# microsoft/hyperspace

Measured on NVIDIA H100. Metric: createIndex rows/sec, higher is better.
Workload: dtype int64

## Files before the change

hyperspace_b200/csrc/device_utils.cuh:

```cuda
#pragma once
#include <cuda_runtime.h>

#include <cstdint>

#ifndef HS_HD
#ifdef __CUDACC__
#define HS_HD __host__ __device__ __forceinline__
#else
#define HS_HD inline
#endif
#endif

namespace hs {

HS_HD uint32_t rotl32(uint32_t x, int r) { return (x << r) | (x >> (32 - r)); }
HS_HD uint32_t mm3_mix_k1(uint32_t k1) {
  k1 *= 0xcc9e2d51u;
  k1 = rotl32(k1, 15);
  k1 *= 0x1b873593u;
  return k1;
}
HS_HD uint32_t mm3_mix_h1(uint32_t h1, uint32_t k1) {
  h1 ^= k1;
  h1 = rotl32(h1, 13);
// ... 199 lines not shown
        "{\n\t"
        ".reg .pred p;\n\t"
        ".reg .b32 t;\n\t"
        "and.b32 t, %2, %3;\n\t"
        "setp.ne.u32 p, t, 0;\n\t"
        "vote.sync.ballot.b32 %0, p, 0xffffffff;\n\t"
        "selp.b32 %1, 0, 0xffffffff, p;\n\t"
        "}"
        : "=r"(m), "=r"(x)
        : "r"(v), "r"(1u << b));
    peers &= m ^ x;
  }
  return peers;
}

__device__ __forceinline__ uint32_t block_exclusive_scan(uint32_t x, uint32_t* warp_sums, uint32_t* total) {
  const unsigned lane = threadIdx.x & 31, warp = threadIdx.x >> 5, nwarps = (blockDim.x + 31) >> 5;
  uint32_t incl = x;
#pragma unroll
  for (int o = 1; o < 32; o <<= 1) {
    uint32_t y = __shfl_up_sync(0xffffffffu, incl, o);
    if (lane >= (unsigned)o) incl += y;
  }
  __syncthreads();
  if (lane == 31) warp_sums[warp] = incl;
  __syncthreads();
  if (warp == 0) {
    uint32_t w = lane < nwarps ? warp_sums[lane] : 0;
    uint32_t wi = w;
#pragma unroll
// ... 17 lines not shown
```

hyperspace_b200/csrc/engine.cu:

```cuda
#include <fcntl.h>
#include <sys/stat.h>
#include <unistd.h>

#include <algorithm>
#include <array>
#include <cmath>
#include <map>
#include <random>

#include "device_utils.cuh"
#include "engine.h"

namespace hs {

std::string make_uuid() {
  std::random_device rd;
  std::mt19937_64 gen(((uint64_t)rd() << 32) ^ rd());
  uint64_t a = gen(), b = gen();
  char buf[40];
  snprintf(buf, sizeof buf, "%08x-%04x-4%03x-%04x-%012llx", (unsigned)(a >> 32), (unsigned)((a >> 16) & 0xffff),
           (unsigned)(a & 0xfff), (unsigned)(0x8000 | ((b >> 48) & 0x3fff)), (unsigned long long)(b & 0xffffffffffffull));
  return buf;
}

// ... 905 lines not shown
    int nbytes = 0, fourth_from_top = 0;
    for (int b = 7, seen = 0; b >= 0; b--)
      if ((varying >> (8 * b)) & 0xff) {
        nbytes++;
        if (++seen == want_bytes) fourth_from_top = b;
      }
    static const bool full_sort_only = getenv("HS_FULL_SORT") != nullptr;
    const RawKeyColumn raw{kc.data.get(), kc.type, kc.width};
    const RawKeyColumn* first_src = from_raw ? &raw : nullptr;
    if (from_raw && (varying == 0 || nrows == 0)) {
      launch_iota_u32(ctx, perm, nrows);
      launch_encode_keys(ctx, kc.data.get(), kc.type, nullptr, nrows, keys, d_or_and.get());
      first_src = nullptr;
    }
    const bool lsd_only = getenv("HS_LSD_SORT") != nullptr;
    if (first_src && !kc.has_nulls && !lsd_only && !full_sort_only) {
      bool local_done = false;
      if (max_bucket <= (uint64_t)kLocalSortCap) {
        segmented_sort_local(ctx, out->bucket_offsets.data(), num_buckets, raw, out->keys.get(), out->perm.get());
        local_done = true;
      } else if (nbytes > 2 && max_bucket <= (uint64_t)(0.85 * 256 * kLocalSortCap)) {
        const int shift = std::max(0, 63 - __builtin_clzll(varying) - 7);
        local_done = segmented_sort_msd_local(ctx, &out->plan, raw, shift, out->keys.get(), out->keys_alt.get(),
                                              out->perm.get(), out->perm_alt.get());
      }
      if (local_done) {
        keys = out->keys.get();
        perm = out->perm.get();
        keys_alt = out->keys_alt.get();
        perm_alt = out->perm_alt.get();
        sort_deferred = defer_settle && nkeys == 1;
        continue;
      }
    }
    if (nbytes > want_bytes && !full_sort_only) {
      const uint64_t high_mask = ~0ull << (8 * fourth_from_top);
      const uint64_t low_mask = ~high_mask;
      segmented_sort_pairs(ctx, &out->plan, keys, keys_alt, perm, perm_alt, varying & high_mask, first_src);
      out->d_fix_flag.alloc(ctx, 1);
// ... 727 lines not shown
```

hyperspace_b200/csrc/kernels.h:

```cpp
#pragma once
#include "hs_common.h"

namespace hs {

struct ChunkDesc {
  const uint8_t* data;
  uint64_t size;
  int64_t num_values;
  int64_t row_base;
  int32_t col;
  int32_t phys_type;
  int32_t max_def;
  int32_t file_index;
  int32_t codec;
  int32_t pad;
};

struct PageDesc {
  const uint8_t* data;
  const uint8_t* dict;
  int64_t first_row;
  int32_t dict_count;
  int32_t size;
  int32_t num_values;
// ... 145 lines not shown
  Buf<uint64_t> seg_start;
  Buf<uint32_t> tile_hist;
  Buf<uint32_t> tile_dst;
  std::vector<uint32_t> h_seg_tile_begin;
};
void build_sort_plan(hs_ctx* ctx, const uint64_t* seg_offsets, int nseg, SortPlan* plan);
struct RawKeyColumn {
  const void* data;
  int type, width;
};
void segmented_sort_pairs(hs_ctx* ctx, SortPlan* plan, uint64_t*& keys, uint64_t*& keys_alt, uint32_t*& vals,
                          uint32_t*& vals_alt, uint64_t bit_mask, const RawKeyColumn* first_pass_source = nullptr);
void launch_fix_runs(hs_ctx* ctx, SortPlan* plan, uint64_t* keys, uint32_t* vals, uint64_t high_mask, uint64_t low_mask,
                     uint32_t max_run, uint32_t* d_flag);
constexpr int kLocalSortCap = 12288;
struct LocalSortItem {
  uint32_t start, count;
};
void segmented_sort_local(hs_ctx* ctx, const uint64_t* seg_offsets, int nseg, const RawKeyColumn& raw, uint64_t* keys,
                          uint32_t* vals);
bool segmented_sort_msd_local(hs_ctx* ctx, SortPlan* plan, const RawKeyColumn& raw, int shift, uint64_t* keys,
                              uint64_t* keys_alt, uint32_t* vals, uint32_t* vals_alt);
void segmented_sort_pass_by_table(hs_ctx* ctx, SortPlan* plan, uint64_t*& keys, uint64_t*& keys_alt, uint32_t*& vals,
                                  uint32_t*& vals_alt, const uint8_t* digits);

struct GatherColumn {
  const void* src;
  const uint64_t* sorted_keys;
  int32_t key_type;
  int32_t width;
  const uint64_t* page_value_offset;
};
void launch_gather_encode(hs_ctx* ctx, const SortTile* tiles, int64_t ntiles, const uint64_t* seg_start,
                          const uint32_t* perm, const GatherColumn& col, const uint32_t* bucket_page_begin,
                          int64_t rows_per_page, uint8_t* arena);
void launch_tile_valid_counts(hs_ctx* ctx, const SortTile* tiles, int64_t ntiles, const uint32_t* perm,
                              const uint8_t* valid, uint32_t* counts);
// ... 79 lines not shown
```

hyperspace_b200/csrc/radix_sort.cu:

```cuda
#include "device_utils.cuh"
#include "kernels.h"

namespace hs {

namespace {

constexpr int kThreads = 512;
constexpr int kWarps = kThreads / 32;
constexpr int kItems = kSortTile / kThreads;
constexpr int kWarpRows = kSortTile / kWarps;
constexpr int kChunkTiles = 128;
constexpr int kHistThreads = 256;

struct SortChunk {
  uint32_t seg;
  uint32_t tile_begin, tile_end;
};

struct DigitShift {
  int shift;
  __device__ __forceinline__ uint32_t operator()(uint64_t key, uint32_t) const { return (uint32_t)(key >> shift) & 255u; }
};
struct DigitTable {
  const uint8_t* table;
  __device__ __forceinline__ uint32_t operator()(uint64_t, uint32_t val) const { return table[val]; }
};

struct SrcPairs {
  const uint64_t* __restrict__ keys;
  const uint32_t* __restrict__ vals;
  __device__ __forceinline__ void load(uint64_t p, uint64_t& k, uint32_t& v) const {
    k = keys[p];
    v = vals[p];
  }
};
template <int TYPE>
struct SrcRaw {
  const void* __restrict__ raw;
  __device__ __forceinline__ void load(uint64_t p, uint64_t& k, uint32_t& v) const {
    const uint64_t r = (TYPE == HS_TYPE_INT64 || TYPE == HS_TYPE_DOUBLE) ? ((const uint64_t*)raw)[p]
                                                                          : (uint64_t)((const uint32_t*)raw)[p];
    k = sort_encode(TYPE, r);
    v = (uint32_t)p;
  }
};

template <typename Src, typename Digit>
__global__ void __launch_bounds__(kHistThreads) k_sort_hist(const SortTile* __restrict__ tiles, Src src, Digit digit,
                                                         uint32_t* __restrict__ tile_hist) {
  __shared__ uint32_t s_hist[256];
  s_hist[threadIdx.x] = 0;
  __syncthreads();
  const SortTile t = tiles[blockIdx.x];
  for (uint32_t i = threadIdx.x; i < t.count; i += kHistThreads) {
    uint64_t k;
    uint32_t v;
    src.load(t.start + i, k, v);
    atomicAdd(&s_hist[digit(k, v)], 1u);
  }
  __syncthreads();
  tile_hist[(size_t)blockIdx.x * 256 + threadIdx.x] = s_hist[threadIdx.x];
}

__global__ void __launch_bounds__(256) k_seg_chunk_sums(const SortChunk* __restrict__ chunks,
                                                         const uint32_t* __restrict__ tile_hist,
                                                         uint32_t* __restrict__ chunk_sums) {
  const SortChunk c = chunks[blockIdx.x];
  uint32_t s = 0;
  for (uint32_t t = c.tile_begin; t < c.tile_end; t++) s += tile_hist[(size_t)t * 256 + threadIdx.x];
  chunk_sums[(size_t)blockIdx.x * 256 + threadIdx.x] = s;
}

__global__ void __launch_bounds__(256) k_seg_scan(const uint32_t* __restrict__ seg_chunk_begin,
                                                   const uint64_t* __restrict__ seg_start,
                                                   uint32_t* __restrict__ chunk_sums, uint32_t* __restrict__ digit_base) {
  __shared__ uint32_t warp_sums[40];
  const uint32_t seg = blockIdx.x;
  const uint32_t c0 = seg_chunk_begin[seg], c1 = seg_chunk_begin[seg + 1];
  uint32_t tot = 0;
  for (uint32_t c = c0; c < c1; c++) {
    const uint32_t v = chunk_sums[(size_t)c * 256 + threadIdx.x];
    chunk_sums[(size_t)c * 256 + threadIdx.x] = tot;
    tot += v;
  }
  const uint32_t dbase = block_exclusive_scan(tot, warp_sums, nullptr) + (uint32_t)seg_start[seg];
  if (digit_base) digit_base[(size_t)seg * 256 + threadIdx.x] = dbase;
  for (uint32_t c = c0; c < c1; c++) chunk_sums[(size_t)c * 256 + threadIdx.x] += dbase;
}

__global__ void __launch_bounds__(1024) k_seg_apply(const SortChunk* __restrict__ chunks,
                                                     const uint32_t* __restrict__ tile_hist,
                                                     uint32_t* __restrict__ tile_dst,
                                                     const uint32_t* __restrict__ chunk_sums) {
  __shared__ uint32_t s_group[4][256];
  const SortChunk c = chunks[blockIdx.x];
  const uint32_t d = threadIdx.x & 255, g = threadIdx.x >> 8;
  const uint32_t n = c.tile_end - c.tile_begin;
  const uint32_t per = (n + 3) / 4;
  const uint32_t t0 = c.tile_begin + min(g * per, n), t1 = c.tile_begin + min((g + 1) * per, n);
  uint32_t s = 0;
#pragma unroll 8
  for (uint32_t t = t0; t < t1; t++) s += tile_hist[(size_t)t * 256 + d];
  s_group[g][d] = s;
  __syncthreads();
  uint32_t run = chunk_sums[(size_t)blockIdx.x * 256 + d];
  for (uint32_t gg = 0; gg < g; gg++) run += s_group[gg][d];
#pragma unroll 8
  for (uint32_t t = t0; t < t1; t++) {
    const uint32_t v = tile_hist[(size_t)t * 256 + d];
    tile_dst[(size_t)t * 256 + d] = run;
    run += v;
  }
}

struct ScatterShared {
  uint64_t keys[kSortTile];
  uint32_t vals[kSortTile];
  uint16_t cnt[kWarps][256];
  uint32_t out_adj[256];
  uint32_t warp_sums[40];
};

template <typename Src, typename Digit>
__global__ void __launch_bounds__(kThreads, 2) k_sort_scatter(const SortTile* __restrict__ tiles, Src src, Digit digit,
                                                               const uint32_t* __restrict__ tile_dst,
                                                               uint64_t* __restrict__ out_keys,
                                                               uint32_t* __restrict__ out_vals) {
  extern __shared__ __align__(16) uint8_t smem_raw[];
  ScatterShared& sm = *reinterpret_cast<ScatterShared*>(smem_raw);
  const uint32_t warp = threadIdx.x >> 5, lane = threadIdx.x & 31;
  const unsigned lt = (1u << lane) - 1;
  {
    uint32_t* z = reinterpret_cast<uint32_t*>(&sm.cnt[0][0]);
#pragma unroll
    for (int i = 0; i < kWarps * 256 / 2 / kThreads; i++) z[threadIdx.x + i * kThreads] = 0;
  }
  const SortTile t = tiles[blockIdx.x];
  uint32_t dst0 = 0;
  if (threadIdx.x < 256) dst0 = tile_dst[(size_t)blockIdx.x * 256 + threadIdx.x];
  const uint32_t first = warp * kWarpRows + lane;
  const uint64_t p0 = t.start + first;
  uint64_t k[kItems];
  uint32_t v[kItems];
  uint32_t bin[kItems];
#pragma unroll
  for (int j = 0; j < kItems; j++) {
    const bool a = first + j * 32 < t.count;
    k[j] = ~0ull;
    v[j] = 0;
    if (a) src.load(p0 + j * 32, k[j], v[j]);
    bin[j] = a ? digit(k[j], v[j]) : 255u;
  }
  __syncthreads();
  uint16_t* cnt = sm.cnt[warp];
  uint32_t rank[kItems];
#pragma unroll
  for (int j = 0; j < kItems; j++) {
    const unsigned peers = match_any_full<8>(bin[j]);
    const uint32_t before = __popc(peers & lt);
    const uint32_t pre = cnt[bin[j]];
    __syncwarp();
    if (before == 0) cnt[bin[j]] = (uint16_t)(pre + __popc(peers));
    __syncwarp();
    rank[j] = pre + before;
  }
  __syncthreads();
  uint32_t total = 0;
  if (threadIdx.x < 256) {
#pragma unroll
    for (int w = 0; w < kWarps; w++) total += sm.cnt[w][threadIdx.x];
  }
  const uint32_t start = block_exclusive_scan(total, sm.warp_sums, nullptr);
  if (threadIdx.x < 256) {
    uint32_t run = start;
#pragma unroll
    for (int w = 0; w < kWarps; w++) {
      const uint16_t c = sm.cnt[w][threadIdx.x];
      sm.cnt[w][threadIdx.x] = (uint16_t)run;
      run += c;
    }
    sm.out_adj[threadIdx.x] = dst0 - start;
  }
  __syncthreads();
#pragma unroll
  for (int j = 0; j < kItems; j++) {
    const uint32_t pos = cnt[bin[j]] + rank[j];
    sm.keys[pos] = k[j];
    sm.vals[pos] = v[j];
// ... 110 lines not shown
      if (b == a) continue;
      const uint32_t va = vals[p + a];
      for (uint32_t c = a; c > b; c--) {
        const uint64_t kc = sk[c - 1];
        sk[c] = kc;
        keys[p + c] = kc;
        vals[p + c] = vals[p + c - 1];
      }
      sk[b] = ka;
      keys[p + b] = ka;
      vals[p + b] = va;
    }
  }
}

constexpr int kLocalThreads = 1024;
constexpr int kLocalWarps = kLocalThreads / 32;
constexpr int kLocalItems = kLocalSortCap / kLocalThreads;
constexpr int kLocalWarpRows = kLocalSortCap / kLocalWarps;
constexpr uint32_t kLocalMaxRun = 64;
static_assert(kLocalSortCap % kLocalThreads == 0 && kLocalSortCap <= 65536, "slot numbers are 16-bit");

struct LocalShared {
  uint64_t keys[kLocalSortCap];
  uint32_t vals[kLocalSortCap];
  uint16_t slot[kLocalSortCap];
  uint16_t cnt[kLocalWarps][256];
  uint32_t warp_sums[40];
  unsigned long long or_bits, and_bits;
  uint32_t long_run;
};

__device__ __forceinline__ void local_pass(LocalShared& sm, uint32_t count, int shift) {
  const uint32_t warp = threadIdx.x >> 5, lane = threadIdx.x & 31;
  const unsigned lt = (1u << lane) - 1;
  {
    uint32_t* z = reinterpret_cast<uint32_t*>(&sm.cnt[0][0]);
#pragma unroll
    for (int i = 0; i < kLocalWarps * 256 / 2 / kLocalThreads; i++) z[threadIdx.x + i * kLocalThreads] = 0;
  }
  const uint32_t first = warp * kLocalWarpRows + lane;
  uint32_t slot_bin[kLocalItems], rank[kLocalItems];
#pragma unroll
  for (int j = 0; j < kLocalItems; j++) {
    const uint32_t pos = first + j * 32;
    const uint32_t s = pos < count ? sm.slot[pos] : pos;
    slot_bin[j] = s << 8 | (pos < count ? (uint32_t)(sm.keys[s] >> shift) & 255u : 255u);
  }
  __syncthreads();
  uint16_t* cnt = sm.cnt[warp];
#pragma unroll
  for (int j = 0; j < kLocalItems; j++) {
    rank[j] = 0;
    if (warp * kLocalWarpRows + j * 32 < count) {
      const uint32_t bin = slot_bin[j] & 255u;
      const unsigned peers = match_any_full<8>(bin);
      const uint32_t before = __popc(peers & lt);
      const uint32_t pre = cnt[bin];
      __syncwarp();
      if (before == 0) cnt[bin] = (uint16_t)(pre + __popc(peers));
      __syncwarp();
      rank[j] = pre + before;
    }
  }
  __syncthreads();
  uint32_t total = 0;
  if (threadIdx.x < 256) {
#pragma unroll
    for (int w = 0; w < kLocalWarps; w++) total += sm.cnt[w][threadIdx.x];
  }
  const uint32_t start = block_exclusive_scan(total, sm.warp_sums, nullptr);
  if (threadIdx.x < 256) {
    uint32_t run = start;
#pragma unroll
    for (int w = 0; w < kLocalWarps; w++) {
      const uint16_t c = sm.cnt[w][threadIdx.x];
      sm.cnt[w][threadIdx.x] = (uint16_t)run;
      run += c;
    }
  }
  __syncthreads();
#pragma unroll
  for (int j = 0; j < kLocalItems; j++)
    if (warp * kLocalWarpRows + j * 32 < count) sm.slot[cnt[slot_bin[j] & 255u] + rank[j]] = (uint16_t)(slot_bin[j] >> 8);
  __syncthreads();
}

template <typename Src>
__global__ void __launch_bounds__(kLocalThreads, 1) k_local_sort(const LocalSortItem* __restrict__ items, Src src,
                                                                 uint64_t* __restrict__ out_keys,
                                                                 uint32_t* __restrict__ out_vals) {
  extern __shared__ __align__(16) uint8_t smem_raw[];
  LocalShared& sm = *reinterpret_cast<LocalShared*>(smem_raw);
  const LocalSortItem it = items[blockIdx.x];
  const uint32_t count = it.count;
  if (threadIdx.x == 0) {
    sm.or_bits = 0;
    sm.and_bits = ~0ull;
    sm.long_run = 0;
  }
  uint64_t k_or = 0, k_and = ~0ull;
  constexpr int kHalf = kLocalItems / 2;
#pragma unroll 1
  for (int h = 0; h < 2; h++) {
    uint64_t k[kHalf];
    uint32_t v[kHalf];
#pragma unroll
    for (int j = 0; j < kHalf; j++) {
      const uint32_t i = (h * kHalf + j) * kLocalThreads + threadIdx.x;
      if (i < count) src.load((uint64_t)it.start + i, k[j], v[j]);
    }
#pragma unroll
    for (int j = 0; j < kHalf; j++) {
      const uint32_t i = (h * kHalf + j) * kLocalThreads + threadIdx.x;
      if (i < count) {
        sm.keys[i] = k[j];
        sm.vals[i] = v[j];
        sm.slot[i] = (uint16_t)i;
        k_or |= k[j];
        k_and &= k[j];
      }
    }
  }
#pragma unroll
  for (int o = 16; o > 0; o >>= 1) {
    k_or |= __shfl_xor_sync(0xffffffffu, k_or, o);
    k_and &= __shfl_xor_sync(0xffffffffu, k_and, o);
  }
  __syncthreads();
  if ((threadIdx.x & 31) == 0) {
    atomicOr(&sm.or_bits, k_or);
    atomicAnd(&sm.and_bits, k_and);
  }
  __syncthreads();
  const uint64_t varying = sm.or_bits ^ sm.and_bits;
  if (varying != 0) {
    const int top = 63 - __clzll((long long)varying);
    int pbits = 1;
    while ((1u << pbits) < 2 * count) pbits++;
    const int ndig = (min(pbits, top + 1) + 7) / 8;
    const int low = max(0, top + 1 - 8 * ndig);
    for (int d = ndig - 1; d >= 0; d--) {
      const int shift = max(0, top + 1 - 8 * (d + 1));
      if ((varying >> shift) & 0xff) local_pass(sm, count, shift);
    }
    const uint64_t high_mask = ~0ull << low;
    if (varying & ~high_mask) {
      for (uint32_t i = threadIdx.x; i < count; i += kLocalThreads) {
        const uint64_t kh = sm.keys[sm.slot[i]] & high_mask;
        if (i > 0 && (sm.keys[sm.slot[i - 1]] & high_mask) == kh) continue;
        if (i + 1 >= count || (sm.keys[sm.slot[i + 1]] & high_mask) != kh) continue;
        uint32_t len = 2;
        while (i + len < count && len <= kLocalMaxRun && (sm.keys[sm.slot[i + len]] & high_mask) == kh) len++;
        if (len > kLocalMaxRun) {
          sm.long_run = 1;
          continue;
        }
        uint16_t* s = sm.slot + i;
        for (uint32_t a = 1; a < len; a++) {
          const uint16_t sa = s[a];
          const uint64_t ka = sm.keys[sa];
          uint32_t b = a;
          while (b > 0 && sm.keys[s[b - 1]] > ka) {
            s[b] = s[b - 1];
            b--;
          }
          s[b] = sa;
        }
      }
      __syncthreads();
      if (sm.long_run) {
        for (uint32_t i = threadIdx.x; i < count; i += kLocalThreads) sm.slot[i] = (uint16_t)i;
        __syncthreads();
        for (int shift = 0; shift < 64; shift += 8)
          if ((varying >> shift) & 0xff) local_pass(sm, count, shift);
      }
    }
  }
  __syncthreads();
#pragma unroll
  for (int j = 0; j < kLocalItems; j++) {
    const uint32_t i = j * kLocalThreads + threadIdx.x;
    if (i < count) {
      const uint32_t s = sm.slot[i];
      out_keys[(uint64_t)it.start + i] = sm.keys[s];
      out_vals[(uint64_t)it.start + i] = sm.vals[s];
    }
  }
}

template <typename Src>
void launch_local_sort(hs_ctx* ctx, const std::vector<LocalSortItem>& items, Src src, uint64_t* out_keys,
                       uint32_t* out_vals) {
  if (items.empty()) return;
  Buf<LocalSortItem> d_items(ctx, items.size());
  copy_h2d(ctx, d_items.get(), items.data(), items.size() * sizeof(LocalSortItem));
  static DeviceOnce attr_once;
  bool& attr = attr_once(ctx->device);
  if (!attr) {
    HS_CUDA(cudaFuncSetAttribute(k_local_sort<Src>, cudaFuncAttributeMaxDynamicSharedMemorySize, (int)sizeof(LocalShared)));
    attr = true;
  }
  KernelScope _ks(ctx, "k_local_sort");
  k_local_sort<Src><<<(unsigned)items.size(), kLocalThreads, sizeof(LocalShared), ctx->stream>>>(d_items.get(), src,
                                                                                                 out_keys, out_vals);
  HS_LAUNCH_CHECK(ctx);
}

template <typename Src, typename Digit>
void run_hist(hs_ctx* ctx, SortPlan* plan, const SortChunk* chunks, int64_t nchunks, const uint32_t* seg_chunk_begin,
              uint32_t* chunk_sums, Src src, Digit digit, uint32_t* digit_base) {
  {
    KernelScope _ks(ctx, "k_sort_hist");
    k_sort_hist<Src, Digit><<<(unsigned)plan->ntiles, kHistThreads, 0, ctx->stream>>>(plan->tiles.get(), src, digit,
                                                                                 plan->tile_hist.get());
    HS_LAUNCH_CHECK(ctx);
  }
  KernelScope _ks(ctx, "k_seg_scan");
  k_seg_chunk_sums<<<(unsigned)nchunks, 256, 0, ctx->stream>>>(chunks, plan->tile_hist.get(), chunk_sums);
  HS_LAUNCH_CHECK(ctx);
  k_seg_scan<<<(unsigned)plan->nseg, 256, 0, ctx->stream>>>(seg_chunk_begin, plan->seg_start.get(), chunk_sums, digit_base);
  HS_LAUNCH_CHECK(ctx);
}

template <typename Src, typename Digit>
void run_scatter(hs_ctx* ctx, SortPlan* plan, const SortChunk* chunks, int64_t nchunks, uint32_t* chunk_sums, Src src,
                 uint64_t* out_keys, uint32_t* out_vals, Digit digit) {
  {
    KernelScope _ks(ctx, "k_seg_scan");
    k_seg_apply<<<(unsigned)nchunks, 1024, 0, ctx->stream>>>(chunks, plan->tile_hist.get(), plan->tile_dst.get(), chunk_sums);
    HS_LAUNCH_CHECK(ctx);
  }
  static DeviceOnce attr_once;
  bool& attr = attr_once(ctx->device);
  if (!attr) {
    HS_CUDA(cudaFuncSetAttribute(k_sort_scatter<Src, Digit>, cudaFuncAttributeMaxDynamicSharedMemorySize,
                                 (int)sizeof(ScatterShared)));
    attr = true;
  }
  KernelScope _ks(ctx, "k_sort_scatter");
  k_sort_scatter<Src, Digit><<<(unsigned)plan->ntiles, kThreads, sizeof(ScatterShared), ctx->stream>>>(
      plan->tiles.get(), src, digit, plan->tile_dst.get(), out_keys, out_vals);
  HS_LAUNCH_CHECK(ctx);
}

template <typename Src, typename Digit>
void run_pass(hs_ctx* ctx, SortPlan* plan, const SortChunk* chunks, int64_t nchunks, const uint32_t* seg_chunk_begin,
              uint32_t* chunk_sums, Src src, uint64_t* out_keys, uint32_t* out_vals, Digit digit) {
  run_hist(ctx, plan, chunks, nchunks, seg_chunk_begin, chunk_sums, src, digit, nullptr);
  run_scatter(ctx, plan, chunks, nchunks, chunk_sums, src, out_keys, out_vals, digit);
}

struct ChunkPlan {
  Buf<SortChunk> chunks;
  Buf<uint32_t> seg_chunk_begin;
  Buf<uint32_t> chunk_sums;
  int64_t nchunks = 0;
};

ChunkPlan build_chunks(hs_ctx* ctx, const std::vector<uint32_t>& seg_tile_begin) {
  ChunkPlan cp;
  const int nseg = (int)seg_tile_begin.size() - 1;
  std::vector<SortChunk> chunks;
  std::vector<uint32_t> scb(nseg + 1);
  for (int s = 0; s < nseg; s++) {
    scb[s] = (uint32_t)chunks.size();
    for (uint32_t t = seg_tile_begin[s]; t < seg_tile_begin[s + 1]; t += kChunkTiles)
      chunks.push_back(SortChunk{(uint32_t)s, t, std::min<uint32_t>(t + kChunkTiles, seg_tile_begin[s + 1])});
  }
  scb[nseg] = (uint32_t)chunks.size();
  cp.nchunks = (int64_t)chunks.size();
  cp.chunks.alloc(ctx, std::max<size_t>(1, chunks.size()));
  cp.seg_chunk_begin.alloc(ctx, scb.size());
  cp.chunk_sums.alloc(ctx, std::max<size_t>(1, chunks.size()) * 256);
  if (!chunks.empty())
    copy_h2d(ctx, cp.chunks.get(), chunks.data(), chunks.size() * sizeof(SortChunk));
  copy_h2d(ctx, cp.seg_chunk_begin.get(), scb.data(), scb.size() * 4);
  return cp;
}

}

__global__ void k_build_tiles(const uint64_t* __restrict__ seg_start, const uint32_t* __restrict__ seg_tile_begin,
                              SortTile* __restrict__ tiles) {
  const uint32_t s = blockIdx.x;
  const uint64_t b = seg_start[s], e = seg_start[s + 1];
  const uint32_t t0 = seg_tile_begin[s], nt = seg_tile_begin[s + 1] - t0;
  for (uint32_t i = threadIdx.x; i < nt; i += blockDim.x) {
    const uint64_t p = b + (uint64_t)i * kSortTile;
// ... 71 lines not shown
    case HS_TYPE_FLOAT: f(SrcRaw<HS_TYPE_FLOAT>{raw.data}); break;
    case HS_TYPE_DOUBLE: f(SrcRaw<HS_TYPE_DOUBLE>{raw.data}); break;
    default: fail(HS_EUNSUPPORTED, "sort: key type %d", raw.type);
  }
}
}

void segmented_sort_local(hs_ctx* ctx, const uint64_t* seg_offsets, int nseg, const RawKeyColumn& raw, uint64_t* keys,
                          uint32_t* vals) {
  std::vector<LocalSortItem> items;
  for (int s = 0; s < nseg; s++) {
    const uint64_t n = seg_offsets[s + 1] - seg_offsets[s];
    if (n > (uint64_t)kLocalSortCap) fail(HS_EINVAL, "segmented_sort_local: segment of %llu rows", (unsigned long long)n);
    if (n) items.push_back(LocalSortItem{(uint32_t)seg_offsets[s], (uint32_t)n});
  }
  with_raw_source(raw, [&](auto src) { launch_local_sort(ctx, items, src, keys, vals); });
}

bool segmented_sort_msd_local(hs_ctx* ctx, SortPlan* plan, const RawKeyColumn& raw, int shift, uint64_t* keys,
                              uint64_t* keys_alt, uint32_t* vals, uint32_t* vals_alt) {
  if (plan->ntiles == 0) return false;
  ChunkPlan cp = build_chunks(ctx, plan->h_seg_tile_begin);
  const size_t nsub = (size_t)plan->nseg * 256;
  Buf<uint32_t> d_base(ctx, nsub);
  const DigitShift digit{shift};
  with_raw_source(raw, [&](auto src) {
    run_hist(ctx, plan, cp.chunks.get(), cp.nchunks, cp.seg_chunk_begin.get(), cp.chunk_sums.get(), src, digit, d_base.get());
  });
  std::vector<uint32_t> base(nsub + 1);
  copy_d2h(ctx, base.data(), d_base.get(), nsub * 4);
  sync_stream(ctx);
  base[nsub] = (uint32_t)plan->n;
  std::vector<LocalSortItem> items;
  for (int s = 0; s < plan->nseg; s++) {
    LocalSortItem cur{base[(size_t)s * 256], 0};
    for (size_t d = (size_t)s * 256; d < (size_t)(s + 1) * 256; d++) {
      const uint32_t sz = base[d + 1] - base[d];
      if (sz > (uint32_t)kLocalSortCap) return false;
      if (cur.count + sz > (uint32_t)kLocalSortCap) {
        items.push_back(cur);
        cur = LocalSortItem{base[d], 0};
      }
      cur.count += sz;
    }
    if (cur.count) items.push_back(cur);
  }
  with_raw_source(raw, [&](auto src) {
    run_scatter(ctx, plan, cp.chunks.get(), cp.nchunks, cp.chunk_sums.get(), src, keys_alt, vals_alt, digit);
  });
  launch_local_sort(ctx, items, SrcPairs{keys_alt, vals_alt}, keys, vals);
  return true;
}

void launch_fix_runs(hs_ctx* ctx, SortPlan* plan, uint64_t* keys, uint32_t* vals, uint64_t high_mask, uint64_t low_mask,
                     uint32_t max_run, uint32_t* d_flag) {
  KernelScope _ks(ctx, "k_fix_runs");
  if (plan->ntiles == 0) return;
  k_fix_runs<<<(unsigned)plan->ntiles, 256, 0, ctx->stream>>>(plan->tiles.get(), plan->seg_start.get(), keys, vals, high_mask,
                                                              low_mask, max_run, d_flag);
  HS_LAUNCH_CHECK(ctx);
}

void segmented_sort_pass_by_table(hs_ctx* ctx, SortPlan* plan, uint64_t*& keys, uint64_t*& keys_alt, uint32_t*& vals,
                                  uint32_t*& vals_alt, const uint8_t* digits) {
  if (plan->ntiles == 0) return;
  ChunkPlan cp = build_chunks(ctx, plan->h_seg_tile_begin);
// ... 8 lines not shown
```

Baseline: 8.002 billion.

## Split MSD local sort into small and large CTA variants with optional 9-bit digit

Templates the local sort kernel on capacity and thread count so that MSD buckets are packed into smaller 6144-row items sorted by a lighter kernel, which can run more CTAs per SM, while oversized buckets go to the large kernel. It also templates the histogram, scan and scatter path on digit width to allow an optional 9-bit MSD digit, and adds cp.async staging helpers plus a reworked local pass using packed words. The aim is better occupancy and load balance in the local-sort phase, at the cost of an extra kernel launch and more complex packing logic.

```diff
diff --git a/hyperspace_b200/csrc/device_utils.cuh b/hyperspace_b200/csrc/device_utils.cuh
--- a/hyperspace_b200/csrc/device_utils.cuh
+++ b/hyperspace_b200/csrc/device_utils.cuh
@@ -237,6 +237,16 @@
   return peers;
 }
 
+__device__ __forceinline__ void cp_async_4(void* smem, const void* gmem) {
+  asm volatile("cp.async.ca.shared.global [%0], [%1], 4;" ::"r"((uint32_t)__cvta_generic_to_shared(smem)), "l"(gmem)
+               : "memory");
+}
+__device__ __forceinline__ void cp_async_8(void* smem, const void* gmem) {
+  asm volatile("cp.async.ca.shared.global [%0], [%1], 8;" ::"r"((uint32_t)__cvta_generic_to_shared(smem)), "l"(gmem)
+               : "memory");
+}
+__device__ __forceinline__ void cp_async_wait_all() { asm volatile("cp.async.wait_all;" ::: "memory"); }
+
 __device__ __forceinline__ uint32_t block_exclusive_scan(uint32_t x, uint32_t* warp_sums, uint32_t* total) {
   const unsigned lane = threadIdx.x & 31, warp = threadIdx.x >> 5, nwarps = (blockDim.x + 31) >> 5;
   uint32_t incl = x;
diff --git a/hyperspace_b200/csrc/engine.cu b/hyperspace_b200/csrc/engine.cu
--- a/hyperspace_b200/csrc/engine.cu
+++ b/hyperspace_b200/csrc/engine.cu
@@ -943,15 +943,18 @@
       first_src = nullptr;
     }
     const bool lsd_only = getenv("HS_LSD_SORT") != nullptr;
+    const bool one_cta = getenv("HS_LOCAL_SORT_1CTA") != nullptr;
+    const bool nine_bit = getenv("HS_LOCAL_SORT_9BIT") != nullptr;
     if (first_src && !kc.has_nulls && !lsd_only && !full_sort_only) {
       bool local_done = false;
       if (max_bucket <= (uint64_t)kLocalSortCap) {
         segmented_sort_local(ctx, out->bucket_offsets.data(), num_buckets, raw, out->keys.get(), out->perm.get());
         local_done = true;
       } else if (nbytes > 2 && max_bucket <= (uint64_t)(0.85 * 256 * kLocalSortCap)) {
-        const int shift = std::max(0, 63 - __builtin_clzll(varying) - 7);
-        local_done = segmented_sort_msd_local(ctx, &out->plan, raw, shift, out->keys.get(), out->keys_alt.get(),
-                                              out->perm.get(), out->perm_alt.get());
+        const int bits = nine_bit && !one_cta && max_bucket / 256 > (uint64_t)kLocalSortSmallCap / 2 ? 9 : 8;
+        const int shift = std::max(0, 63 - __builtin_clzll(varying) + 1 - bits);
+        local_done = segmented_sort_msd_local(ctx, &out->plan, raw, shift, bits, one_cta, out->keys.get(),
+                                              out->keys_alt.get(), out->perm.get(), out->perm_alt.get());
       }
       if (local_done) {
         keys = out->keys.get();
diff --git a/hyperspace_b200/csrc/kernels.h b/hyperspace_b200/csrc/kernels.h
--- a/hyperspace_b200/csrc/kernels.h
+++ b/hyperspace_b200/csrc/kernels.h
@@ -183,13 +183,14 @@
 void launch_fix_runs(hs_ctx* ctx, SortPlan* plan, uint64_t* keys, uint32_t* vals, uint64_t high_mask, uint64_t low_mask,
                      uint32_t max_run, uint32_t* d_flag);
 constexpr int kLocalSortCap = 12288;
+constexpr int kLocalSortSmallCap = 6144;
 struct LocalSortItem {
   uint32_t start, count;
 };
 void segmented_sort_local(hs_ctx* ctx, const uint64_t* seg_offsets, int nseg, const RawKeyColumn& raw, uint64_t* keys,
                           uint32_t* vals);
-bool segmented_sort_msd_local(hs_ctx* ctx, SortPlan* plan, const RawKeyColumn& raw, int shift, uint64_t* keys,
-                              uint64_t* keys_alt, uint32_t* vals, uint32_t* vals_alt);
+bool segmented_sort_msd_local(hs_ctx* ctx, SortPlan* plan, const RawKeyColumn& raw, int shift, int bits, bool one_cta,
+                              uint64_t* keys, uint64_t* keys_alt, uint32_t* vals, uint32_t* vals_alt);
 void segmented_sort_pass_by_table(hs_ctx* ctx, SortPlan* plan, uint64_t*& keys, uint64_t*& keys_alt, uint32_t*& vals,
                                   uint32_t*& vals_alt, const uint8_t* digits);
 
diff --git a/hyperspace_b200/csrc/radix_sort.cu b/hyperspace_b200/csrc/radix_sort.cu
--- a/hyperspace_b200/csrc/radix_sort.cu
+++ b/hyperspace_b200/csrc/radix_sort.cu
@@ -17,11 +17,17 @@
   uint32_t tile_begin, tile_end;
 };
 
-struct DigitShift {
+template <int BITS>
+struct DigitBits {
+  static constexpr int kBits = BITS;
   int shift;
-  __device__ __forceinline__ uint32_t operator()(uint64_t key, uint32_t) const { return (uint32_t)(key >> shift) & 255u; }
+  __device__ __forceinline__ uint32_t operator()(uint64_t key, uint32_t) const {
+    return (uint32_t)(key >> shift) & ((1u << BITS) - 1);
+  }
 };
+using DigitShift = DigitBits<8>;
 struct DigitTable {
+  static constexpr int kBits = 8;
   const uint8_t* table;
   __device__ __forceinline__ uint32_t operator()(uint64_t, uint32_t val) const { return table[val]; }
 };
@@ -33,23 +39,39 @@
     k = keys[p];
     v = vals[p];
   }
+  __device__ __forceinline__ void stage(uint64_t p, uint64_t* sk, uint32_t* sv) const {
+    cp_async_8(sk, keys + p);
+    cp_async_4(sv, vals + p);
+  }
+  __device__ __forceinline__ uint64_t finish(uint64_t, uint64_t* sk, uint32_t*) const { return *sk; }
 };
 template <int TYPE>
 struct SrcRaw {
+  static constexpr bool kWide = TYPE == HS_TYPE_INT64 || TYPE == HS_TYPE_DOUBLE;
   const void* __restrict__ raw;
   __device__ __forceinline__ void load(uint64_t p, uint64_t& k, uint32_t& v) const {
-    const uint64_t r = (TYPE == HS_TYPE_INT64 || TYPE == HS_TYPE_DOUBLE) ? ((const uint64_t*)raw)[p]
-                                                                          : (uint64_t)((const uint32_t*)raw)[p];
+    const uint64_t r = kWide ? ((const uint64_t*)raw)[p] : (uint64_t)((const uint32_t*)raw)[p];
     k = sort_encode(TYPE, r);
     v = (uint32_t)p;
+  }
+  __device__ __forceinline__ void stage(uint64_t p, uint64_t* sk, uint32_t*) const {
+    if (kWide) cp_async_8(sk, (const uint64_t*)raw + p);
+    else cp_async_4(sk, (const uint32_t*)raw + p);
+  }
+  __device__ __forceinline__ uint64_t finish(uint64_t p, uint64_t* sk, uint32_t* sv) const {
+    const uint64_t k = sort_encode(TYPE, kWide ? *sk : (uint64_t)*(const uint32_t*)sk);
+    *sk = k;
+    *sv = (uint32_t)p;
+    return k;
   }
 };
 
 template <typename Src, typename Digit>
 __global__ void __launch_bounds__(kHistThreads) k_sort_hist(const SortTile* __restrict__ tiles, Src src, Digit digit,
                                                          uint32_t* __restrict__ tile_hist) {
-  __shared__ uint32_t s_hist[256];
-  s_hist[threadIdx.x] = 0;
+  constexpr int kBins = 1 << Digit::kBits;
+  __shared__ uint32_t s_hist[kBins];
+  for (int b = threadIdx.x; b < kBins; b += kHistThreads) s_hist[b] = 0;
   __syncthreads();
   const SortTile t = tiles[blockIdx.x];
   for (uint32_t i = threadIdx.x; i < t.count; i += kHistThreads) {
@@ -59,65 +81,70 @@
     atomicAdd(&s_hist[digit(k, v)], 1u);
   }
   __syncthreads();
-  tile_hist[(size_t)blockIdx.x * 256 + threadIdx.x] = s_hist[threadIdx.x];
-}
-
-__global__ void __launch_bounds__(256) k_seg_chunk_sums(const SortChunk* __restrict__ chunks,
-                                                         const uint32_t* __restrict__ tile_hist,
-                                                         uint32_t* __restrict__ chunk_sums) {
+  for (int b = threadIdx.x; b < kBins; b += kHistThreads) tile_hist[(size_t)blockIdx.x * kBins + b] = s_hist[b];
+}
+
+template <int BINS>
+__global__ void __launch_bounds__(BINS) k_seg_chunk_sums(const SortChunk* __restrict__ chunks,
+                                                          const uint32_t* __restrict__ tile_hist,
+                                                          uint32_t* __restrict__ chunk_sums) {
   const SortChunk c = chunks[blockIdx.x];
   uint32_t s = 0;
-  for (uint32_t t = c.tile_begin; t < c.tile_end; t++) s += tile_hist[(size_t)t * 256 + threadIdx.x];
-  chunk_sums[(size_t)blockIdx.x * 256 + threadIdx.x] = s;
-}
-
-__global__ void __launch_bounds__(256) k_seg_scan(const uint32_t* __restrict__ seg_chunk_begin,
-                                                   const uint64_t* __restrict__ seg_start,
-                                                   uint32_t* __restrict__ chunk_sums, uint32_t* __restrict__ digit_base) {
+  for (uint32_t t = c.tile_begin; t < c.tile_end; t++) s += tile_hist[(size_t)t * BINS + threadIdx.x];
+  chunk_sums[(size_t)blockIdx.x * BINS + threadIdx.x] = s;
+}
+
+template <int BINS>
+__global__ void __launch_bounds__(BINS) k_seg_scan(const uint32_t* __restrict__ seg_chunk_begin,
+                                                    const uint64_t* __restrict__ seg_start,
+                                                    uint32_t* __restrict__ chunk_sums, uint32_t* __restrict__ digit_base) {
   __shared__ uint32_t warp_sums[40];
   const uint32_t seg = blockIdx.x;
   const uint32_t c0 = seg_chunk_begin[seg], c1 = seg_chunk_begin[seg + 1];
   uint32_t tot = 0;
   for (uint32_t c = c0; c < c1; c++) {
-    const uint32_t v = chunk_sums[(size_t)c * 256 + threadIdx.x];
-    chunk_sums[(size_t)c * 256 + threadIdx.x] = tot;
+    const uint32_t v = chunk_sums[(size_t)c * BINS + threadIdx.x];
+    chunk_sums[(size_t)c * BINS + threadIdx.x] = tot;
     tot += v;
   }
   const uint32_t dbase = block_exclusive_scan(tot, warp_sums, nullptr) + (uint32_t)seg_start[seg];
-  if (digit_base) digit_base[(size_t)seg * 256 + threadIdx.x] = dbase;
-  for (uint32_t c = c0; c < c1; c++) chunk_sums[(size_t)c * 256 + threadIdx.x] += dbase;
-}
-
+  if (digit_base) digit_base[(size_t)seg * BINS + threadIdx.x] = dbase;
+  for (uint32_t c = c0; c < c1; c++) chunk_sums[(size_t)c * BINS + threadIdx.x] += dbase;
+}
+
+template <int BINS>
 __global__ void __launch_bounds__(1024) k_seg_apply(const SortChunk* __restrict__ chunks,
                                                      const uint32_t* __restrict__ tile_hist,
                                                      uint32_t* __restrict__ tile_dst,
                                                      const uint32_t* __restrict__ chunk_sums) {
-  __shared__ uint32_t s_group[4][256];
+  constexpr uint32_t kGroups = 1024 / BINS;
+  __shared__ uint32_t s_group[kGroups][BINS];
   const SortChunk c = chunks[blockIdx.x];
-  const uint32_t d = threadIdx.x & 255, g = threadIdx.x >> 8;
+  const uint32_t d = threadIdx.x % BINS, g = threadIdx.x / BINS;
   const uint32_t n = c.tile_end - c.tile_begin;
-  const uint32_t per = (n + 3) / 4;
+  const uint32_t per = (n + kGroups - 1) / kGroups;
   const uint32_t t0 = c.tile_begin + min(g * per, n), t1 = c.tile_begin + min((g + 1) * per, n);
   uint32_t s = 0;
 #pragma unroll 8
-  for (uint32_t t = t0; t < t1; t++) s += tile_hist[(size_t)t * 256 + d];
+  for (uint32_t t = t0; t < t1; t++) s += tile_hist[(size_t)t * BINS + d];
   s_group[g][d] = s;
   __syncthreads();
-  uint32_t run = chunk_sums[(size_t)blockIdx.x * 256 + d];
+  uint32_t run = chunk_sums[(size_t)blockIdx.x * BINS + d];
   for (uint32_t gg = 0; gg < g; gg++) run += s_group[gg][d];
 #pragma unroll 8
   for (uint32_t t = t0; t < t1; t++) {
-    const uint32_t v = tile_hist[(size_t)t * 256 + d];
-    tile_dst[(size_t)t * 256 + d] = run;
+    const uint32_t v = tile_hist[(size_t)t * BINS + d];
+    tile_dst[(size_t)t * BINS + d] = run;
     run += v;
   }
 }
 
+template <int BINS>
 struct ScatterShared {
   uint64_t keys[kSortTile];
   uint32_t vals[kSortTile];
-  uint16_t cnt[kWarps][256];
-  uint32_t out_adj[256];
+  uint16_t cnt[kWarps][BINS];
+  uint32_t out_adj[BINS];
   uint32_t warp_sums[40];
 };
 
@@ -126,18 +153,20 @@
                                                                const uint32_t* __restrict__ tile_dst,
                                                                uint64_t* __restrict__ out_keys,
                                                                uint32_t* __restrict__ out_vals) {
+  constexpr int kBins = 1 << Digit::kBits;
+  static_assert(kBins <= kThreads, "one thread per digit");
   extern __shared__ __align__(16) uint8_t smem_raw[];
-  ScatterShared& sm = *reinterpret_cast<ScatterShared*>(smem_raw);
+  ScatterShared<kBins>& sm = *reinterpret_cast<ScatterShared<kBins>*>(smem_raw);
   const uint32_t warp = threadIdx.x >> 5, lane = threadIdx.x & 31;
   const unsigned lt = (1u << lane) - 1;
   {
     uint32_t* z = reinterpret_cast<uint32_t*>(&sm.cnt[0][0]);
 #pragma unroll
-    for (int i = 0; i < kWarps * 256 / 2 / kThreads; i++) z[threadIdx.x + i * kThreads] = 0;
+    for (int i = 0; i < kWarps * kBins / 2 / kThreads; i++) z[threadIdx.x + i * kThreads] = 0;
   }
   const SortTile t = tiles[blockIdx.x];
   uint32_t dst0 = 0;
-  if (threadIdx.x < 256) dst0 = tile_dst[(size_t)blockIdx.x * 256 + threadIdx.x];
+  if (threadIdx.x < kBins) dst0 = tile_dst[(size_t)blockIdx.x * kBins + threadIdx.x];
   const uint32_t first = warp * kWarpRows + lane;
   const uint64_t p0 = t.start + first;
   uint64_t k[kItems];
@@ -149,14 +178,14 @@
     k[j] = ~0ull;
     v[j] = 0;
     if (a) src.load(p0 + j * 32, k[j], v[j]);
-    bin[j] = a ? digit(k[j], v[j]) : 255u;
+    bin[j] = a ? digit(k[j], v[j]) : (uint32_t)(kBins - 1);
   }
   __syncthreads();
   uint16_t* cnt = sm.cnt[warp];
   uint32_t rank[kItems];
 #pragma unroll
   for (int j = 0; j < kItems; j++) {
-    const unsigned peers = match_any_full<8>(bin[j]);
+    const unsigned peers = match_any_full<Digit::kBits>(bin[j]);
     const uint32_t before = __popc(peers & lt);
     const uint32_t pre = cnt[bin[j]];
     __syncwarp();
@@ -166,12 +195,12 @@
   }
   __syncthreads();
   uint32_t total = 0;
-  if (threadIdx.x < 256) {
+  if (threadIdx.x < kBins) {
 #pragma unroll
     for (int w = 0; w < kWarps; w++) total += sm.cnt[w][threadIdx.x];
   }
   const uint32_t start = block_exclusive_scan(total, sm.warp_sums, nullptr);
-  if (threadIdx.x < 256) {
+  if (threadIdx.x < kBins) {
     uint32_t run = start;
 #pragma unroll
     for (int w = 0; w < kWarps; w++) {
@@ -312,51 +341,60 @@
   }
 }
 
-constexpr int kLocalThreads = 1024;
-constexpr int kLocalWarps = kLocalThreads / 32;
-constexpr int kLocalItems = kLocalSortCap / kLocalThreads;
-constexpr int kLocalWarpRows = kLocalSortCap / kLocalWarps;
 constexpr uint32_t kLocalMaxRun = 64;
-static_assert(kLocalSortCap % kLocalThreads == 0 && kLocalSortCap <= 65536, "slot numbers are 16-bit");
-
+
+template <int CAP, int THREADS>
 struct LocalShared {
-  uint64_t keys[kLocalSortCap];
-  uint32_t vals[kLocalSortCap];
-  uint16_t slot[kLocalSortCap];
-  uint16_t cnt[kLocalWarps][256];
+  static constexpr int kWarps = THREADS / 32;
+  static constexpr int kItems = CAP / THREADS;
+  static constexpr int kWarpRows = CAP / kWarps;
+  static_assert(CAP % THREADS == 0 && CAP <= 16384, "16-bit slots; two 8-bit digits give twice as many prefixes as rows");
+  uint64_t keys[CAP];
+  uint32_t vals[CAP];
+  uint32_t word[CAP];
+  uint16_t cnt[kWarps][256];
   uint32_t warp_sums[40];
   unsigned long long or_bits, and_bits;
   uint32_t long_run;
+  uint32_t start;
 };
 
-__device__ __forceinline__ void local_pass(LocalShared& sm, uint32_t count, int shift) {
+template <bool BY_KEY, int CAP, int THREADS>
+__device__ __forceinline__ void local_pass(LocalShared<CAP, THREADS>& sm, uint32_t count, int sh) {
+  using LS = LocalShared<CAP, THREADS>;
   const uint32_t warp = threadIdx.x >> 5, lane = threadIdx.x & 31;
   const unsigned lt = (1u << lane) - 1;
   {
     uint32_t* z = reinterpret_cast<uint32_t*>(&sm.cnt[0][0]);
 #pragma unroll
-    for (int i = 0; i < kLocalWarps * 256 / 2 / kLocalThreads; i++) z[threadIdx.x + i * kLocalThreads] = 0;
-  }
-  const uint32_t first = warp * kLocalWarpRows + lane;
-  uint32_t slot_bin[kLocalItems], rank[kLocalItems];
-#pragma unroll
-  for (int j = 0; j < kLocalItems; j++) {
+    for (int i = 0; i < LS::kWarps * 256 / 2 / THREADS; i++) z[threadIdx.x + i * THREADS] = 0;
+  }
+  const uint32_t first = warp * LS::kWarpRows + lane;
+  uint32_t r[LS::kItems], rank[LS::kItems];
+#pragma unroll
+  for (int j = 0; j < LS::kItems; j++) {
     const uint32_t pos = first + j * 32;
-    const uint32_t s = pos < count ? sm.slot[pos] : pos;
-    slot_bin[j] = s << 8 | (pos < count ? (uint32_t)(sm.keys[s] >> shift) & 255u : 255u);
-  }
+    if (BY_KEY) {
+      const uint32_t s = pos < count ? sm.word[pos] : pos;
+      r[j] = s << 8 | (pos < count ? (uint32_t)(sm.keys[s] >> sh) & 255u : 255u);
+    } else {
+      const uint32_t w = pos < count ? sm.word[pos] : ~0u;
+      r[j] = __funnelshift_r(w, w, sh);
+    }
+  }
+  const auto bin = [](uint32_t x) { return x & 255u; };
   __syncthreads();
   uint16_t* cnt = sm.cnt[warp];
 #pragma unroll
-  for (int j = 0; j < kLocalItems; j++) {
+  for (int j = 0; j < LS::kItems; j++) {
     rank[j] = 0;
-    if (warp * kLocalWarpRows + j * 32 < count) {
-      const uint32_t bin = slot_bin[j] & 255u;
-      const unsigned peers = match_any_full<8>(bin);
+    if (warp * LS::kWarpRows + j * 32 < count) {
+      const uint32_t b = bin(r[j]);
+      const unsigned peers = match_any_full<8>(b);
       const uint32_t before = __popc(peers & lt);
-      const uint32_t pre = cnt[bin];
+      const uint32_t pre = cnt[b];
       __syncwarp();
-      if (before == 0) cnt[bin] = (uint16_t)(pre + __popc(peers));
+      if (before == 0) cnt[b] = (uint16_t)(pre + __popc(peers));
       __syncwarp();
       rank[j] = pre + before;
     }
@@ -365,13 +403,13 @@
   uint32_t total = 0;
   if (threadIdx.x < 256) {
 #pragma unroll
-    for (int w = 0; w < kLocalWarps; w++) total += sm.cnt[w][threadIdx.x];
+    for (int w = 0; w < LS::kWarps; w++) total += sm.cnt[w][threadIdx.x];
   }
   const uint32_t start = block_exclusive_scan(total, sm.warp_sums, nullptr);
   if (threadIdx.x < 256) {
     uint32_t run = start;
 #pragma unroll
-    for (int w = 0; w < kLocalWarps; w++) {
+    for (int w = 0; w < LS::kWarps; w++) {
       const uint16_t c = sm.cnt[w][threadIdx.x];
       sm.cnt[w][threadIdx.x] = (uint16_t)run;
       run += c;
@@ -379,45 +417,40 @@
   }
   __syncthreads();
 #pragma unroll
-  for (int j = 0; j < kLocalItems; j++)
-    if (warp * kLocalWarpRows + j * 32 < count) sm.slot[cnt[slot_bin[j] & 255u] + rank[j]] = (uint16_t)(slot_bin[j] >> 8);
-  __syncthreads();
-}
-
-template <typename Src>
-__global__ void __launch_bounds__(kLocalThreads, 1) k_local_sort(const LocalSortItem* __restrict__ items, Src src,
-                                                                 uint64_t* __restrict__ out_keys,
-                                                                 uint32_t* __restrict__ out_vals) {
+  for (int j = 0; j < LS::kItems; j++)
+    if (warp * LS::kWarpRows + j * 32 < count) sm.word[cnt[bin(r[j])] + rank[j]] = BY_KEY ? r[j] >> 8 : __funnelshift_l(r[j], r[j], sh);
+  __syncthreads();
+}
+
+template <int CAP, int THREADS, int MIN_BLOCKS, typename Src>
+__global__ void __launch_bounds__(THREADS, MIN_BLOCKS) k_local_sort(const LocalSortItem* __restrict__ items, Src src,
+                                                                    uint64_t* __restrict__ out_keys,
+                                                                    uint32_t* __restrict__ out_vals) {
+  using LS = LocalShared<CAP, THREADS>;
   extern __shared__ __align__(16) uint8_t smem_raw[];
-  LocalShared& sm = *reinterpret_cast<LocalShared*>(smem_raw);
+  LS& sm = *reinterpret_cast<LS*>(smem_raw);
   const LocalSortItem it = items[blockIdx.x];
   const uint32_t count = it.count;
   if (threadIdx.x == 0) {
     sm.or_bits = 0;
     sm.and_bits = ~0ull;
     sm.long_run = 0;
-  }
+    sm.start = it.start;
+  }
+#pragma unroll 1
+  for (int j = 0; j < LS::kItems; j++) {
+    const uint32_t i = j * THREADS + threadIdx.x;
+    if (i < count) src.stage((uint64_t)it.start + i, &sm.keys[i], &sm.vals[i]);
+  }
+  cp_async_wait_all();
   uint64_t k_or = 0, k_and = ~0ull;
-  constexpr int kHalf = kLocalItems / 2;
-#pragma unroll 1
-  for (int h = 0; h < 2; h++) {
-    uint64_t k[kHalf];
-    uint32_t v[kHalf];
-#pragma unroll
-    for (int j = 0; j < kHalf; j++) {
-      const uint32_t i = (h * kHalf + j) * kLocalThreads + threadIdx.x;
-      if (i < count) src.load((uint64_t)it.start + i, k[j], v[j]);
-    }
-#pragma unroll
-    for (int j = 0; j < kHalf; j++) {
-      const uint32_t i = (h * kHalf + j) * kLocalThreads + threadIdx.x;
-      if (i < count) {
-        sm.keys[i] = k[j];
-        sm.vals[i] = v[j];
-        sm.slot[i] = (uint16_t)i;
-        k_or |= k[j];
-        k_and &= k[j];
-      }
+#pragma unroll
+  for (int j = 0; j < LS::kItems; j++) {
+    const uint32_t i = j * THREADS + threadIdx.x;
+    if (i < count) {
+      const uint64_t k = src.finish((uint64_t)it.start + i, &sm.keys[i], &sm.vals[i]);
+      k_or |= k;
+      k_and &= k;
     }
   }
 #pragma unroll
@@ -432,76 +465,92 @@
   }
   __syncthreads();
   const uint64_t varying = sm.or_bits ^ sm.and_bits;
+  int top = 0, ndig = 0, low = 0;
   if (varying != 0) {
-    const int top = 63 - __clzll((long long)varying);
+    top = 63 - __clzll((long long)varying);
     int pbits = 1;
     while ((1u << pbits) < 2 * count) pbits++;
-    const int ndig = (min(pbits, top + 1) + 7) / 8;
-    const int low = max(0, top + 1 - 8 * ndig);
-    for (int d = ndig - 1; d >= 0; d--) {
-      const int shift = max(0, top + 1 - 8 * (d + 1));
-      if ((varying >> shift) & 0xff) local_pass(sm, count, shift);
-    }
-    const uint64_t high_mask = ~0ull << low;
-    if (varying & ~high_mask) {
-      for (uint32_t i = threadIdx.x; i < count; i += kLocalThreads) {
-        const uint64_t kh = sm.keys[sm.slot[i]] & high_mask;
-        if (i > 0 && (sm.keys[sm.slot[i - 1]] & high_mask) == kh) continue;
-        if (i + 1 >= count || (sm.keys[sm.slot[i + 1]] & high_mask) != kh) continue;
+    ndig = (min(pbits, top + 1) + 7) / 8;
+    low = max(0, top + 1 - 8 * ndig);
+  }
+  for (uint32_t i = threadIdx.x; i < count; i += THREADS) sm.word[i] = (uint32_t)(sm.keys[i] >> low) << 16 | i;
+  __syncthreads();
+  const auto varying_bits = [&sm]() {
+    return *(volatile unsigned long long*)&sm.or_bits ^ *(volatile unsigned long long*)&sm.and_bits;
+  };
+  for (int d = ndig - 1; d >= 0; d--) {
+    const int shift = max(0, top + 1 - 8 * (d + 1));
+    if ((varying_bits() >> shift) & 0xff) local_pass<false>(sm, count, 16 + shift - low);
+  }
+  {
+    if (varying_bits() & ((1ull << low) - 1)) {
+      for (uint32_t i = threadIdx.x; i < count; i += THREADS) {
+        const uint32_t ph = sm.word[i] >> 16;
+        if (i > 0 && sm.word[i - 1] >> 16 == ph) continue;
+        if (i + 1 >= count || sm.word[i + 1] >> 16 != ph) continue;
         uint32_t len = 2;
-        while (i + len < count && len <= kLocalMaxRun && (sm.keys[sm.slot[i + len]] & high_mask) == kh) len++;
+        while (i + len < count && len <= kLocalMaxRun && sm.word[i + len] >> 16 == ph) len++;
         if (len > kLocalMaxRun) {
           sm.long_run = 1;
           continue;
         }
-        uint16_t* s = sm.slot + i;
+        uint32_t* w = sm.word + i;
         for (uint32_t a = 1; a < len; a++) {
-          const uint16_t sa = s[a];
-          const uint64_t ka = sm.keys[sa];
+          const uint32_t wa = w[a];
+          const uint64_t ka = sm.keys[wa & 0xffffu];
           uint32_t b = a;
-          while (b > 0 && sm.keys[s[b - 1]] > ka) {
-            s[b] = s[b - 1];
+          while (b > 0 && sm.keys[w[b - 1] & 0xffffu] > ka) {
+            w[b] = w[b - 1];
             b--;
           }
-          s[b] = sa;
+          w[b] = wa;
         }
       }
       __syncthreads();
       if (sm.long_run) {
-        for (uint32_t i = threadIdx.x; i < count; i += kLocalThreads) sm.slot[i] = (uint16_t)i;
+        for (uint32_t i = threadIdx.x; i < count; i += THREADS) sm.word[i] = i;
         __syncthreads();
         for (int shift = 0; shift < 64; shift += 8)
-          if ((varying >> shift) & 0xff) local_pass(sm, count, shift);
+          if ((varying_bits() >> shift) & 0xff) local_pass<true>(sm, count, shift);
       }
     }
   }
   __syncthreads();
-#pragma unroll
-  for (int j = 0; j < kLocalItems; j++) {
-    const uint32_t i = j * kLocalThreads + threadIdx.x;
+  const uint64_t start = *(volatile uint32_t*)&sm.start;
+#pragma unroll
+  for (int j = 0; j < LS::kItems; j++) {
+    const uint32_t i = j * THREADS + threadIdx.x;
     if (i < count) {
-      const uint32_t s = sm.slot[i];
-      out_keys[(uint64_t)it.start + i] = sm.keys[s];
-      out_vals[(uint64_t)it.start + i] = sm.vals[s];
-    }
-  }
-}
-
-template <typename Src>
+      const uint32_t s = sm.word[i] & 0xffffu;
+      out_keys[start + i] = sm.keys[s];
+      out_vals[start + i] = sm.vals[s];
+    }
+  }
+}
+
+#define HS_LOCAL_LARGE kLocalSortCap, 1024, 1
+#define HS_LOCAL_SMALL kLocalSortSmallCap, 512, 2
+
+template <int CAP, int THREADS, int MIN_BLOCKS, typename Src>
 void launch_local_sort(hs_ctx* ctx, const std::vector<LocalSortItem>& items, Src src, uint64_t* out_keys,
                        uint32_t* out_vals) {
   if (items.empty()) return;
+  const auto kernel = k_local_sort<CAP, THREADS, MIN_BLOCKS, Src>;
+  constexpr int smem = (int)sizeof(LocalShared<CAP, THREADS>);
   Buf<LocalSortItem> d_items(ctx, items.size());
   copy_h2d(ctx, d_items.get(), items.data(), items.size() * sizeof(LocalSortItem));
   static DeviceOnce attr_once;
   bool& attr = attr_once(ctx->device);
   if (!attr) {
-    HS_CUDA(cudaFuncSetAttribute(k_local_sort<Src>, cudaFuncAttributeMaxDynamicSharedMemorySize, (int)sizeof(LocalShared)));
+    HS_CUDA(cudaFuncSetAttribute(kernel, cudaFuncAttributeMaxDynamicSharedMemorySize, smem));
+    int per_sm = 0;
+    HS_CUDA(cudaOccupancyMaxActiveBlocksPerMultiprocessor(&per_sm, kernel, THREADS, smem));
+    if (per_sm < MIN_BLOCKS)
+      fail(HS_ECUDA, "k_local_sort<%d>: %d CTAs per SM (%d B of shared memory), %d expected", CAP, per_sm, smem, MIN_BLOCKS);
     attr = true;
   }
   KernelScope _ks(ctx, "k_local_sort");
-  k_local_sort<Src><<<(unsigned)items.size(), kLocalThreads, sizeof(LocalShared), ctx->stream>>>(d_items.get(), src,
-                                                                                                 out_keys, out_vals);
+  kernel<<<(unsigned)items.size(), THREADS, smem, ctx->stream>>>(d_items.get(), src, out_keys, out_vals);
   HS_LAUNCH_CHECK(ctx);
 }
 
@@ -514,30 +563,34 @@
                                                                                  plan->tile_hist.get());
     HS_LAUNCH_CHECK(ctx);
   }
+  constexpr int kBins = 1 << Digit::kBits;
   KernelScope _ks(ctx, "k_seg_scan");
-  k_seg_chunk_sums<<<(unsigned)nchunks, 256, 0, ctx->stream>>>(chunks, plan->tile_hist.get(), chunk_sums);
+  k_seg_chunk_sums<kBins><<<(unsigned)nchunks, kBins, 0, ctx->stream>>>(chunks, plan->tile_hist.get(), chunk_sums);
   HS_LAUNCH_CHECK(ctx);
-  k_seg_scan<<<(unsigned)plan->nseg, 256, 0, ctx->stream>>>(seg_chunk_begin, plan->seg_start.get(), chunk_sums, digit_base);
+  k_seg_scan<kBins><<<(unsigned)plan->nseg, kBins, 0, ctx->stream>>>(seg_chunk_begin, plan->seg_start.get(), chunk_sums,
+                                                                    digit_base);
   HS_LAUNCH_CHECK(ctx);
 }
 
 template <typename Src, typename Digit>
 void run_scatter(hs_ctx* ctx, SortPlan* plan, const SortChunk* chunks, int64_t nchunks, uint32_t* chunk_sums, Src src,
                  uint64_t* out_keys, uint32_t* out_vals, Digit digit) {
+  constexpr int kBins = 1 << Digit::kBits;
   {
     KernelScope _ks(ctx, "k_seg_scan");
-    k_seg_apply<<<(unsigned)nchunks, 1024, 0, ctx->stream>>>(chunks, plan->tile_hist.get(), plan->tile_dst.get(), chunk_sums);
+    k_seg_apply<kBins><<<(unsigned)nchunks, 1024, 0, ctx->stream>>>(chunks, plan->tile_hist.get(), plan->tile_dst.get(),
+                                                                    chunk_sums);
     HS_LAUNCH_CHECK(ctx);
   }
   static DeviceOnce attr_once;
   bool& attr = attr_once(ctx->device);
   if (!attr) {
     HS_CUDA(cudaFuncSetAttribute(k_sort_scatter<Src, Digit>, cudaFuncAttributeMaxDynamicSharedMemorySize,
-                                 (int)sizeof(ScatterShared)));
+                                 (int)sizeof(ScatterShared<kBins>)));
     attr = true;
   }
   KernelScope _ks(ctx, "k_sort_scatter");
-  k_sort_scatter<Src, Digit><<<(unsigned)plan->ntiles, kThreads, sizeof(ScatterShared), ctx->stream>>>(
+  k_sort_scatter<Src, Digit><<<(unsigned)plan->ntiles, kThreads, sizeof(ScatterShared<kBins>), ctx->stream>>>(
       plan->tiles.get(), src, digit, plan->tile_dst.get(), out_keys, out_vals);
   HS_LAUNCH_CHECK(ctx);
 }
@@ -556,7 +609,7 @@
   int64_t nchunks = 0;
 };
 
-ChunkPlan build_chunks(hs_ctx* ctx, const std::vector<uint32_t>& seg_tile_begin) {
+ChunkPlan build_chunks(hs_ctx* ctx, const std::vector<uint32_t>& seg_tile_begin, int bins = 256) {
   ChunkPlan cp;
   const int nseg = (int)seg_tile_begin.size() - 1;
   std::vector<SortChunk> chunks;
@@ -570,7 +623,7 @@
   cp.nchunks = (int64_t)chunks.size();
   cp.chunks.alloc(ctx, std::max<size_t>(1, chunks.size()));
   cp.seg_chunk_begin.alloc(ctx, scb.size());
-  cp.chunk_sums.alloc(ctx, std::max<size_t>(1, chunks.size()) * 256);
+  cp.chunk_sums.alloc(ctx, std::max<size_t>(1, chunks.size()) * bins);
   if (!chunks.empty())
     copy_h2d(ctx, cp.chunks.get(), chunks.data(), chunks.size() * sizeof(SortChunk));
   copy_h2d(ctx, cp.seg_chunk_begin.get(), scb.data(), scb.size() * 4);
@@ -672,16 +725,22 @@
     if (n > (uint64_t)kLocalSortCap) fail(HS_EINVAL, "segmented_sort_local: segment of %llu rows", (unsigned long long)n);
     if (n) items.push_back(LocalSortItem{(uint32_t)seg_offsets[s], (uint32_t)n});
   }
-  with_raw_source(raw, [&](auto src) { launch_local_sort(ctx, items, src, keys, vals); });
-}
-
-bool segmented_sort_msd_local(hs_ctx* ctx, SortPlan* plan, const RawKeyColumn& raw, int shift, uint64_t* keys,
-                              uint64_t* keys_alt, uint32_t* vals, uint32_t* vals_alt) {
-  if (plan->ntiles == 0) return false;
-  ChunkPlan cp = build_chunks(ctx, plan->h_seg_tile_begin);
-  const size_t nsub = (size_t)plan->nseg * 256;
+  with_raw_source(raw, [&](auto src) { launch_local_sort<HS_LOCAL_LARGE>(ctx, items, src, keys, vals); });
+}
+
+namespace {
+template <typename Digit>
+bool msd_local(hs_ctx* ctx, SortPlan* plan, const RawKeyColumn& raw, Digit digit, bool one_cta, uint64_t* keys,
+               uint64_t* keys_alt, uint32_t* vals, uint32_t* vals_alt) {
+  constexpr int kBits = Digit::kBits;
+  const size_t ntiles_bins = (size_t)plan->ntiles << kBits;
+  if (plan->tile_hist.size() < ntiles_bins) {
+    plan->tile_hist.alloc(ctx, ntiles_bins);
+    plan->tile_dst.alloc(ctx, ntiles_bins);
+  }
+  ChunkPlan cp = build_chunks(ctx, plan->h_seg_tile_begin, 1 << kBits);
+  const size_t nsub = (size_t)plan->nseg << kBits;
   Buf<uint32_t> d_base(ctx, nsub);
-  const DigitShift digit{shift};
   with_raw_source(raw, [&](auto src) {
     run_hist(ctx, plan, cp.chunks.get(), cp.nchunks, cp.seg_chunk_begin.get(), cp.chunk_sums.get(), src, digit, d_base.get());
   });
@@ -689,25 +748,46 @@
   copy_d2h(ctx, base.data(), d_base.get(), nsub * 4);
   sync_stream(ctx);
   base[nsub] = (uint32_t)plan->n;
-  std::vector<LocalSortItem> items;
+  const uint32_t pack_cap = one_cta ? kLocalSortCap : kLocalSortSmallCap;
+  std::vector<LocalSortItem> small, large;
+  std::vector<LocalSortItem>& packed = one_cta ? large : small;
   for (int s = 0; s < plan->nseg; s++) {
-    LocalSortItem cur{base[(size_t)s * 256], 0};
-    for (size_t d = (size_t)s * 256; d < (size_t)(s + 1) * 256; d++) {
+    const size_t d0 = (size_t)s << kBits, d1 = (size_t)(s + 1) << kBits;
+    LocalSortItem cur{base[d0], 0};
+    for (size_t d = d0; d < d1; d++) {
       const uint32_t sz = base[d + 1] - base[d];
       if (sz > (uint32_t)kLocalSortCap) return false;
-      if (cur.count + sz > (uint32_t)kLocalSortCap) {
-        items.push_back(cur);
+      if (sz > pack_cap) {
+        if (cur.count) packed.push_back(cur);
+        large.push_back(LocalSortItem{base[d], sz});
+        cur = LocalSortItem{base[d + 1], 0};
+        continue;
+      }
+      if (cur.count + sz > pack_cap) {
+        packed.push_back(cur);
         cur = LocalSortItem{base[d], 0};
       }
       cur.count += sz;
     }
-    if (cur.count) items.push_back(cur);
+    if (cur.count) packed.push_back(cur);
   }
   with_raw_source(raw, [&](auto src) {
     run_scatter(ctx, plan, cp.chunks.get(), cp.nchunks, cp.chunk_sums.get(), src, keys_alt, vals_alt, digit);
   });
-  launch_local_sort(ctx, items, SrcPairs{keys_alt, vals_alt}, keys, vals);
+  launch_local_sort<HS_LOCAL_SMALL>(ctx, small, SrcPairs{keys_alt, vals_alt}, keys, vals);
+  launch_local_sort<HS_LOCAL_LARGE>(ctx, large, SrcPairs{keys_alt, vals_alt}, keys, vals);
   return true;
+}
+}
+
+bool segmented_sort_msd_local(hs_ctx* ctx, SortPlan* plan, const RawKeyColumn& raw, int shift, int bits, bool one_cta,
+                              uint64_t* keys, uint64_t* keys_alt, uint32_t* vals, uint32_t* vals_alt) {
+  if (plan->ntiles == 0) return false;
+  switch (bits) {
+    case 8: return msd_local(ctx, plan, raw, DigitBits<8>{shift}, one_cta, keys, keys_alt, vals, vals_alt);
+    case 9: return msd_local(ctx, plan, raw, DigitBits<9>{shift}, one_cta, keys, keys_alt, vals, vals_alt);
+    default: fail(HS_EINVAL, "segmented_sort_msd_local: %d-bit digit", bits);
+  }
 }
 
 void launch_fix_runs(hs_ctx* ctx, SortPlan* plan, uint64_t* keys, uint32_t* vals, uint64_t high_mask, uint64_t low_mask,
```

Result: no change. 8.072 billion (median of 6 runs) (+0.9%).
